# ishine/StyleTTS-ZS

Measured on AMD Instinct MI355X. Metric: synthesized audio-sec/sec (whole job) + p50 utterance latency, 3-s ref -> 5-s target, higher is better.
Workload: dtype bf16; 1 GPU; configs[2]: batch 64/GPU, 5-s targets, 2-step distilled style diffusion, CFG 5; global_batch=64, seq_len=200, parallelism=dp1 (utterance shards), spec=v0, graph=True, branch_streams=False, streams=2, schedule=pipe, stagger=0

## Files before the change

include/stzs.h:

```cpp
#ifndef STZS_H
#define STZS_H

#include <stddef.h>
#include <stdint.h>

#ifdef __cplusplus
extern "C" {
#endif

#define STZS_OK 0
#define STZS_EINVAL (-1)
#define STZS_ESHAPE (-2)
#define STZS_EDTYPE (-3)
#define STZS_EHIP (-4)

enum { STZS_F32 = 0, STZS_BF16 = 1, STZS_I32 = 2, STZS_F8 = 3  };
enum { STZS_ACT_NONE = 0, STZS_ACT_LEAKY = 1, STZS_ACT_SNAKE = 2, STZS_ACT_GELU = 3, STZS_ACT_SILU = 4 };
enum { STZS_PRO_NONE = 0, STZS_PRO_ADAIN = 1 };
#define STZS_CONV_A_DMA 8

int stzs_init(int device);
const char* stzs_strerror(int code);
int stzs_version(void);

// ... 17 lines not shown
    int32_t in_dtype, out_dtype;
    int32_t pro_mode, pro_act, epi_act, flags;
    float pro_cscale, pro_slope, epi_slope, alpha, beta, pad_f;
    void* stat_part;
    int64_t stat_ld;
    const float* x_scale;
    const float* w_scale;
    void* splitk_ws;
    unsigned int* splitk_ctr;
    int32_t splitk;
    int32_t pad_sk;
    const float* pro_part;
    int64_t pro_ld;
    int32_t pro_nch, pro_T;
    float pro_eps, pad_pp;
} stzs_conv_args;
size_t stzs_conv_splitk_workspace(int64_t rows, int32_t co_pad, int32_t splitk);
#define STZS_CONV_STAT_ROWS 64
#define STZS_CONV_W_LANE16 16
#define STZS_CONV_W_NARROW32 32
#define STZS_CONV_W_F32 64
#define STZS_CONV_LINEAR_IDS 128
#define STZS_CONV_W_FRAG32 256
#define STZS_CONV_W_X3 1024
#define STZS_CONV_ROWS 2048
#define STZS_CONV_UPS_NOISE 4096
#define STZS_CONV_MRFV_NARROW 8192
#define STZS_CONV_W_FRAG32X3 16384
#define STZS_CONV_MRFV_T128 32768
#define STZS_CONV_RING 65536
// ... 331 lines not shown
```

styletts-zs_amd/csrc/dispatch.hip:

```cpp
#include "common.hpp"

int stzs_conv1d_core(const stzs_conv_args* a, void* stream);
int stzs_mrfv_conv_launch(const stzs_conv_args& a, hipStream_t s);
int stzs_rows_gemm_launch(const stzs_conv_args& a, hipStream_t s);
int stzs_mrfx_conv_launch(const stzs_conv_args& a, hipStream_t s);

int stzs_mrfv_trio_launch(const stzs_conv_args* a, hipStream_t s);
int stzs_conv_pair_launch(const stzs_conv_args* a, hipStream_t s);

namespace {

int frag32_checks(const stzs_conv_args* a) {
    if (!a->x || !a->w || !a->y) return STZS_EINVAL;
    if (a->flags & (STZS_CONV_W_LANE16 | STZS_CONV_W_NARROW32 | STZS_CONV_W_F32 | STZS_CONV_A_DMA)) return STZS_EINVAL;
    if (a->B <= 0 || a->T_in <= 0 || a->T_out <= 0 || a->Ci <= 0 || a->Co <= 0 || a->dil <= 0) return STZS_ESHAPE;
    if (a->ci_pad < a->Ci || a->co_pad < a->Co) return STZS_ESHAPE;
    if (a->ldx % 8 || a->bsx % 8 || a->ldx < ((a->Ci + 7) / 8) * 8) return STZS_ESHAPE;
    if (!stzs_aligned(a->x, 16) || !stzs_aligned(a->w, 16) || !stzs_aligned(a->y, 16)) return STZS_EINVAL;
    if (a->pro_mode == STZS_PRO_ADAIN && (!a->pro_mean || !a->pro_rstd || !a->pro_gb)) return STZS_EINVAL;
    if (a->in_dtype == STZS_F8 || a->x_scale) return STZS_EDTYPE;
    if (a->splitk > 1) return STZS_EINVAL;
    if (a->stat_part && !stzs_aligned(a->stat_part, 8)) return STZS_EINVAL;
    return STZS_OK;
}

}

extern "C" int stzs_conv1d_group(const stzs_conv_args* a, int n, void* stream) {
    if (!a || n < 1 || n > 3) return STZS_EINVAL;
    if (n == 3 && !a[0].pro_part && !a[1].pro_part && !a[2].pro_part && (a[0].flags & STZS_CONV_W_FRAG32) &&
        (a[1].flags & STZS_CONV_W_FRAG32) && (a[2].flags & STZS_CONV_W_FRAG32) && !(a[0].flags & STZS_CONV_W_FRAG32X3) &&
        !(a[1].flags & STZS_CONV_W_FRAG32X3) && !(a[2].flags & STZS_CONV_W_FRAG32X3) && a[0].ups <= 0 && a[1].ups <= 0 &&
        a[2].ups <= 0 && frag32_checks(&a[0]) == STZS_OK && frag32_checks(&a[1]) == STZS_OK &&
        frag32_checks(&a[2]) == STZS_OK) {
        const int rc = stzs_mrfv_trio_launch(a, reinterpret_cast<hipStream_t>(stream));
        if (rc == STZS_OK) return 1;
        if (rc != STZS_ESHAPE) return rc;
    }
    if (n == 2 && !a[0].pro_part == !a[1].pro_part) {
        const int rc = stzs_conv_pair_launch(a, reinterpret_cast<hipStream_t>(stream));
        if (rc == STZS_OK) return 1;
        if (rc != STZS_ESHAPE) return rc;
    }
    for (int i = 0; i < n; ++i) {
        const int rc = stzs_conv1d(&a[i], stream);
        if (rc != STZS_OK) return rc;
    }
    return n;
}

extern "C" int stzs_conv1d(const stzs_conv_args* a, void* stream) {
    if (a && a->pro_part && (a->flags & (STZS_CONV_W_FRAG32X3 | STZS_CONV_W_FRAG32 | STZS_CONV_ROWS))) return STZS_EINVAL;
    if (a && (a->flags & STZS_CONV_W_FRAG32X3)) {
        if (!a->x || !a->w || !a->y) return STZS_EINVAL;
        if (a->flags & (STZS_CONV_W_LANE16 | STZS_CONV_W_NARROW32 | STZS_CONV_W_F32 | STZS_CONV_W_X3 | STZS_CONV_A_DMA |
                        STZS_CONV_W_FRAG32 | STZS_CONV_ROWS | STZS_CONV_UPS_NOISE))
            return STZS_EINVAL;
        if (a->B <= 0 || a->T_in <= 0 || a->T_out <= 0 || a->Ci <= 0 || a->Co <= 0 || a->dil <= 0) return STZS_ESHAPE;
        if (a->ci_pad < a->Ci || a->co_pad < a->Co || a->ldx < ((a->Ci + 7) / 8) * 8) return STZS_ESHAPE;
        if (!stzs_aligned(a->w, 16)) return STZS_EINVAL;
        if (a->pro_mode == STZS_PRO_ADAIN && (!a->pro_mean || !a->pro_rstd || !a->pro_gb)) return STZS_EINVAL;
        if (a->in_dtype == STZS_F8 || a->x_scale) return STZS_EDTYPE;
        if (a->splitk > 1) return STZS_EINVAL;
        if (a->stat_part && !stzs_aligned(a->stat_part, 8)) return STZS_EINVAL;
        return stzs_mrfx_conv_launch(*a, reinterpret_cast<hipStream_t>(stream));
    }
// ... 17 lines not shown
```

styletts-zs_amd/csrc/lnrows.hip:

```cpp
#include "conv_common.hpp"

namespace {

constexpr int LR_ROWS = 16;

STZS_DEV float sum16(float v) {
    v += dpp_f32<0x128>(v);
    v += dpp_f32<0x124>(v);
    v += dpp_f32<0x122>(v);
    v += dpp_f32<0x121>(v);
    return v;
}

template <typename TI, typename TOut, int NK, int EACT>
__global__ __launch_bounds__(NTHR) void ln_rows(const stzs_conv_args a, const stzs_rowln_args ln) {
    constexpr int K = NK * 32;
    constexpr int PITCH = K * 2 + 16;
    constexpr int NV = NK / 4;
    __shared__ __attribute__((aligned(16))) unsigned char lds[LR_ROWS * PITCH];
    const int tid = threadIdx.x, lane = tid & 63, wave = tid >> 6;
    const int nR = ln.R;
    const int r0 = blockIdx.y * LR_ROWS;
    const int ct = blockIdx.x * 4 + wave;
    const bool wact = ct * 16 < a.Co;
// ... 264 lines not shown
    const int wpg = (!split && nks <= 16) ? env_wpg : 4;
    if (a->in_dtype == STZS_BF16 && a->out_dtype == STZS_BF16) k = pick_plain<bf16_t, bf16_t>(nks, split, a->epi_act, wpg);
    else if (a->in_dtype == STZS_BF16 && a->out_dtype == STZS_F32) k = pick_plain<bf16_t, float>(nks, split, a->epi_act, wpg);
    else if (a->in_dtype == STZS_F32 && a->out_dtype == STZS_F32) k = pick_plain<float, float>(nks, split, a->epi_act, wpg);
    else return STZS_EDTYPE;
    if (!k) return STZS_EINVAL;
    dim3 grid((unsigned)((a->Co + 16 * wpg - 1) / (16 * wpg)), (unsigned)(((long)a->B * a->T_in + LR_ROWS - 1) / LR_ROWS),
              (unsigned)Z);
    hipLaunchKernelGGL(reinterpret_cast<void (*)(stzs_conv_args)>(k), grid, dim3(64 * wpg), 0, s, *a);
    STZS_LAUNCH_CHECK();
    return STZS_OK;
}

extern "C" int stzs_ln_linear(const stzs_conv_args* a, const stzs_rowln_args* ln, void* stream) {
    if (!a || !a->w || !a->y) return STZS_EINVAL;
    if (!ln) return plain_launch(a, reinterpret_cast<hipStream_t>(stream));
    if (!ln->x || ln->lens) return STZS_EINVAL;
    const bool lin = a->ks == 1 && a->stride == 1 && a->pad == 0 && a->ups == 0 && a->T_in == a->T_out &&
                     a->pro_mode == STZS_PRO_NONE && a->pro_act == STZS_ACT_NONE && !a->stat_part && !a->x_scale &&
                     !a->res && !a->gate && a->splitk <= 1;
    if (!lin || (a->flags & (STZS_CONV_W_LANE16 | STZS_CONV_W_NARROW32 | STZS_CONV_W_F32 | STZS_CONV_W_X3 |
                             STZS_CONV_W_FRAG32 | STZS_CONV_UPS_NOISE)))
        return STZS_EINVAL;
    if (a->B <= 0 || a->T_in <= 0 || a->Co <= 0 || a->Co > a->co_pad || a->co_pad % 128) return STZS_ESHAPE;
    const int C = ln->C, nk = C / 32;
    if (C != a->Ci || C != a->ci_pad || C % 32 || (nk != 4 && nk != 8 && nk != 16)) return STZS_ESHAPE;
    if ((long)ln->R != (long)a->B * a->T_in || ln->R >= (1 << 22) - LR_ROWS || ln->ldx % 8 || ln->gdiv <= 0 ||
        !stzs_aligned(ln->x, 16))
        return STZS_ESHAPE;
    if ((ln->G && (ln->gs % 8 || !stzs_aligned(ln->G, 32))) || (ln->Bt && (ln->bs % 8 || !stzs_aligned(ln->Bt, 32))))
// ... 17 lines not shown
```

styletts-zs_amd/csrc/mrfv.hip:

```cpp
#include "mrfv_kernel.hpp"

namespace {

template <int PACT, bool HR, bool HA>
void (*pick(int ks, bool one, bool al, bool wide, bool t64))(stzs_conv_args) {
    if (wide) return al ? pick_ks<PACT, HR, HA, 0, true, 2>(ks) : pick_ks<PACT, HR, HA, 0, false, 2>(ks);
    static_assert(PACT == STZS_ACT_SNAKE, "the single-chunk forms are the Snake (MRF) convs");
    if (one) return stzs_mrfv_pick_n1(ks, HR, HA, al, t64);
    if (t64)
        return al ? pick_ks<PACT, HR, HA, 0, true, 1, 64>(ks) : pick_ks<PACT, HR, HA, 0, false, 1, 64>(ks);
    return al ? pick_ks<PACT, HR, HA, 0, true>(ks) : pick_ks<PACT, HR, HA, 0, false>(ks);
}

}

int stzs_ups_conv_launch(const stzs_conv_args& a, hipStream_t s);

namespace {

int mrfv_shape(const stzs_conv_args& a) {
    const int rows_in = 128 + (a.ks - 1) * a.dil;
    if (a.stride != 1 || a.cic != 128 || a.ci_pad % 128 || a.Co % 8 || a.co_pad % BCO || rows_in > 16 * sb_rows(a.ks) ||
        a.in_dtype != STZS_BF16 || a.out_dtype != STZS_BF16 || a.gate || a.epi_act != STZS_ACT_NONE || a.ups ||
        a.refl || a.ldy % 8 || a.bsy % 8 || (a.res && (a.ldr % 8 || a.bsr % 8 || a.res_tdiv <= 0)) ||
// ... 37 lines not shown
    void (*k)(stzs_conv_args, stzs_conv_args, stzs_conv_args) =
        a[0].ci_pad == 128 ? stzs_mrfv_trio_pick_n1(R) : (R ? mrfv_trio<true, 0, 64> : mrfv_trio<false, 0, 64>);
    (void)hipFuncSetAttribute((const void*)k, hipFuncAttributeMaxDynamicSharedMemorySize, (int)lds);
    dim3 grid((unsigned)a[0].B * (unsigned)((a[0].T_out + 63) / 64), a[0].co_pad / BCO, 3);
    hipLaunchKernelGGL(k, grid, dim3(NTH), lds, s, a[0], a[1], a[2]);
    STZS_LAUNCH_CHECK();
    return STZS_OK;
}

__attribute__((visibility("hidden"))) int stzs_mrfv_conv_launch(const stzs_conv_args& a, hipStream_t s) {
    if (a.ups > 0) return stzs_ups_conv_launch(a, s);
    {
        const int rc = mrfv_shape(a);
        if (rc != STZS_OK) return rc;
    }
    void (*k)(stzs_conv_args) = nullptr;
    const bool R = a.res != nullptr, A = a.acc_in != nullptr;
    bool blk_wide = false, blk_t64 = false;
    bool wide, t64;
    snake_form(a, wide, t64);
    const long wide_tiles = (long)a.B * ((a.T_out + 127) / 128) * (a.co_pad / (2 * BCO));
    const long tiles128 = (long)a.B * ((a.T_out + 127) / 128) * (a.co_pad / BCO);
    if (a.pro_act == STZS_ACT_SNAKE) {
        const bool one = a.ci_pad == 128;
        const bool al = a.alpha != 1.f;
        k = R ? (A ? pick<STZS_ACT_SNAKE, true, true>(a.ks, one, al, wide, t64) : pick<STZS_ACT_SNAKE, true, false>(a.ks, one, al, wide, t64))
              : (A ? pick<STZS_ACT_SNAKE, false, true>(a.ks, one, al, wide, t64) : pick<STZS_ACT_SNAKE, false, false>(a.ks, one, al, wide, t64));
    } else if (!A && a.ks == 1 && a.pro_act == STZS_ACT_NONE && a.pro_mode == STZS_PRO_NONE && !a.stat_part) {
        blk_wide = a.ci_pad > 128 && a.co_pad % (2 * BCO) == 0 && wide_tiles >= 2 * stzs_cu_count() &&
                   !(a.flags & STZS_CONV_MRFV_NARROW);
        blk_t64 = !blk_wide && tiles128 < 4 * stzs_cu_count() && !(a.flags & STZS_CONV_MRFV_T128);
// ... 10 lines not shown
        blk_t64 = !blk_wide && t64_blk > 0 && tiles128 < t64_blk * stzs_cu_count() && !(a.flags & STZS_CONV_MRFV_T128);
        if (a.pro_act == STZS_ACT_LEAKY)
            k = blk_wide ? (R ? mrfv_conv<STZS_ACT_LEAKY, true, false, 3, 0, true, 2> : mrfv_conv<STZS_ACT_LEAKY, false, false, 3, 0, true, 2>)
              : blk_t64 ? (R ? mrfv_conv<STZS_ACT_LEAKY, true, false, 3, 0, true, 1, 64> : mrfv_conv<STZS_ACT_LEAKY, false, false, 3, 0, true, 1, 64>)
                         : (R ? mrfv_conv<STZS_ACT_LEAKY, true, false, 3, 0, true> : mrfv_conv<STZS_ACT_LEAKY, false, false, 3, 0, true>);
        else if (a.pro_act == STZS_ACT_NONE)
            k = blk_wide ? (R ? mrfv_conv<STZS_ACT_NONE, true, false, 3, 0, true, 2> : mrfv_conv<STZS_ACT_NONE, false, false, 3, 0, true, 2>)
              : blk_t64 ? (R ? mrfv_conv<STZS_ACT_NONE, true, false, 3, 0, true, 1, 64> : mrfv_conv<STZS_ACT_NONE, false, false, 3, 0, true, 1, 64>)
                         : (R ? mrfv_conv<STZS_ACT_NONE, true, false, 3, 0, true> : mrfv_conv<STZS_ACT_NONE, false, false, 3, 0, true>);
    }
    if (!k) return STZS_ESHAPE;
    const int BTk = (t64 || blk_t64) ? 64 : 128;
    const size_t ldsk = mrfv_lds(BTk + (a.ks - 1) * a.dil);
    (void)hipFuncSetAttribute((const void*)k, hipFuncAttributeMaxDynamicSharedMemorySize, (int)ldsk);
    dim3 grid((unsigned)a.B * (unsigned)((a.T_out + BTk - 1) / BTk), a.co_pad / (wide || blk_wide ? 2 * BCO : BCO));
    hipLaunchKernelGGL(k, grid, dim3(NTH), ldsk, s, a);
    STZS_LAUNCH_CHECK();
    return STZS_OK;
}
```

styletts-zs_amd/csrc/mrfv_kernel.hpp:

```cpp
#pragma once
#include "common.hpp"

#include <type_traits>

#ifndef STZS_MRFV_OCC
#define STZS_MRFV_OCC 2
#endif
#ifndef STZS_MRFV_OCC1
#define STZS_MRFV_OCC1 3
#endif

namespace {

constexpr int NTH = 256;
constexpr int BCO = 128;
#ifndef STZS_MRFV_P
#define STZS_MRFV_P 288
#endif
constexpr int P = STZS_MRFV_P;
constexpr int sb_rows(int ks) { return ks == 1 ? 8 : ks == 3 ? 9 : (ks == 7 ? 10 : 12); }
constexpr int sb_rows64(int ks) { return ks == 1 ? 4 : ks == 3 ? 5 : (ks == 7 ? 6 : 8); }
constexpr int SB_MAX = 12;
constexpr int CS_BYTES = 5 * 128 * 4;
constexpr bool CS_IN_PAD = P >= 288;
// ... 20 lines not shown
    for (int i = 0; i < N; ++i) asm volatile("v_add_f32_dpp %0, %0, %0 row_mirror row_mask:0xf bank_mask:0xf" : "+v"(x[i]));
}

#ifdef STZS_MRFV_PROF
__device__ unsigned long long g_mprof[8 * 16384];
#define MPROF(i, v)                                                                    \
    if (threadIdx.x == 0) {                                                            \
        const unsigned wg_ = blockIdx.y * gridDim.x + blockIdx.x;                     \
        if (wg_ < 16384) g_mprof[wg_ * 8 + (i)] = (v);                                 \
    }
#else
#define MPROF(i, v)
#endif

template <int PACT, bool HR, bool HA, int KS, int NCH, bool AL, int WPW = 1, int BT = 128>
STZS_DEV void mrfv_body(const stzs_conv_args a) {
    static_assert(WPW == 1 || (WPW == 2 && NCH != 1), "the wide form is for multi-chunk inputs");
    static_assert(BT == 128 || (BT == 64 && WPW == 1), "64-row tiles: narrow form");
    MPROF(5, __builtin_amdgcn_s_memrealtime())
    MPROF(0, __builtin_amdgcn_s_memtime())
    MPROF(7, (unsigned long long)__builtin_amdgcn_s_getreg(4 | (31 << 11)) |
                 ((unsigned long long)__builtin_amdgcn_s_getreg(0x14 | (3 << 11)) << 32))
    constexpr int NA = 2 * WPW;
    constexpr int MT = BT / 16;
    extern __shared__ __attribute__((aligned(16))) unsigned char smem[];
    constexpr int NKC = KS * 4;
    const int dil = a.dil;
    const int rows_in = BT + (KS - 1) * dil;
    auto cs = [&](int i) { return cs_at(smem, rows_in, i); };
    const int tid = threadIdx.x, lane = tid & 63, wave = tid >> 6;
    const int tpb = (a.T_out + BT - 1) / BT;
    const int nx = gridDim.x;
    const int lin = (a.flags & STZS_CONV_LINEAR_IDS) ? blockIdx.y * nx + blockIdx.x
                                                      : xcd_remap(blockIdx.y * nx + blockIdx.x, nx * gridDim.y);
    const int by = lin / nx, bx = lin - by * nx;
    const int bq = bx / tpb;
    const int t0 = (bx - bq * tpb) * BT;
    const int nchunk = NCH ? NCH : a.ci_pad >> 7;
    constexpr int SB = BT == 128 ? sb_rows(KS) : sb_rows64(KS);
    const int ct = WPW == 1 ? by : by * 2 + (wave >> 1);
    const int ow0 = WPW == 1 ? wave : (wave & 1) * 2;
    const bf16x8* Wf = reinterpret_cast<const bf16x8*>(a.w) + ((long)ct * nchunk * NKC) * 512 + ow0 * 128 + lane;
    auto wload = [&](bf16x8 (&w)[NA], int kk) {
        const bf16x8* p = Wf + (long)kk * 512;
#pragma unroll
        for (int j = 0; j < NA; ++j) w[j] = p[64 * j];
    };
    f32x4 acc[NA][MT];

// ... 283 lines not shown
                    Pp[2 * i + 1] = sq[i];
                }
            }
        }
    }
    }
#ifdef STZS_MRFV_PROF
    MPROF(3, __builtin_amdgcn_s_memtime())
    asm volatile("s_waitcnt vmcnt(0)" ::: "memory");
    MPROF(4, __builtin_amdgcn_s_memtime())
    MPROF(6, __builtin_amdgcn_s_memrealtime())
#endif
}

template <int PACT, bool HR, bool HA, int KS, int NCH, bool AL, int WPW = 1, int BT = 128>
__global__ __launch_bounds__(NTH, NCH == 1 ? STZS_MRFV_OCC1 : STZS_MRFV_OCC) void mrfv_conv(const stzs_conv_args a) {
    mrfv_body<PACT, HR, HA, KS, NCH, AL, WPW, BT>(a);
}

template <bool HR, int NCH, int BT>
__global__ __launch_bounds__(NTH, NCH == 1 ? STZS_MRFV_OCC1 : STZS_MRFV_OCC) void mrfv_trio(const stzs_conv_args a3,
                                                                                        const stzs_conv_args a7,
                                                                                        const stzs_conv_args a11) {
    if (blockIdx.z == 0)
        mrfv_body<STZS_ACT_SNAKE, HR, false, 11, NCH, false, 1, BT>(a11);
    else if (blockIdx.z == 1)
        mrfv_body<STZS_ACT_SNAKE, HR, false, 7, NCH, false, 1, BT>(a7);
    else
        mrfv_body<STZS_ACT_SNAKE, HR, false, 3, NCH, false, 1, BT>(a3);
}

template <int PACT, bool HR, bool HA, int NCH, bool AL, int WPW = 1, int BT = 128>
void (*pick_ks(int ks))(stzs_conv_args) {
    switch (ks) {
        case 3: return mrfv_conv<PACT, HR, HA, 3, NCH, AL, WPW, BT>;
        case 7: return mrfv_conv<PACT, HR, HA, 7, NCH, AL, WPW, BT>;
        case 11: return mrfv_conv<PACT, HR, HA, 11, NCH, AL, WPW, BT>;
        default: return nullptr;
    }
}

}

using mrfv_kfn = void (*)(stzs_conv_args);
mrfv_kfn stzs_mrfv_pick_n1(int ks, bool hr, bool ha, bool al, bool t64);
using mrfv_trio_kfn = void (*)(stzs_conv_args, stzs_conv_args, stzs_conv_args);
mrfv_trio_kfn stzs_mrfv_trio_pick_n1(bool hr);
```

styletts-zs_amd/csrc/norm.hip:

```cpp
#include "common.hpp"
#include "rowln.hpp"

namespace {

constexpr int STAT_ROWS = 256;
constexpr int STAT_CG = 32;

template <typename T>
__global__ __launch_bounds__(256) void chan_stats_partial(const stzs_stats_args a, int nchunk) {
    __shared__ float red[8][STAT_CG * 8][2];
    const int tid = threadIdx.x, tx = tid & 31, ty = tid >> 5;
    const int chunk = blockIdx.x, b = blockIdx.y;
    const int cv = blockIdx.z * STAT_CG + tx;
    const int c = cv * 8;
    float s[8], q[8];
#pragma unroll
    for (int j = 0; j < 8; ++j) s[j] = q[j] = 0.f;
    const int r0 = chunk * STAT_ROWS, r1 = min(a.T, r0 + STAT_ROWS);
    const T* X = reinterpret_cast<const T*>(a.x) + (long)b * a.bs;
    if (c < a.C) {
        int r = r0 + ty;
        for (; r + 24 < r1; r += 32) {
            float v[4][8];
#pragma unroll
// ... 26 lines not shown
    const int cg = blockIdx.z * STAT_CG * 8 + cl;
    if (cg < a.C) {
        float ss = 0.f, qq = 0.f;
#pragma unroll
        for (int y = 0; y < 8; ++y) {
            ss += red[y][cl][0];
            qq += red[y][cl][1];
        }
        float* P = reinterpret_cast<float*>(a.partial);
        const long o = (((long)b * nchunk + chunk) * a.C + cg) * 2;
        P[o] = ss;
        P[o + 1] = qq;
    }
}

constexpr int FIN_CH = 32;
STZS_DEV void stats_final_body(const stzs_stats_args a, int nchunk, int b, int by) {
    __shared__ double red[8][FIN_CH][2];
    const int tid = threadIdx.x, cl = tid & (FIN_CH - 1), g = tid >> 5;
    const int c = by * FIN_CH + cl;
    double s = 0.0, q = 0.0;
    if (c < a.C) {
        const float2* P = reinterpret_cast<const float2*>(a.partial) + (long)b * nchunk * a.C + c;
        int k = g;
        for (; k + 24 < nchunk; k += 32) {
            float2 v[4];
#pragma unroll
            for (int u = 0; u < 4; ++u) v[u] = P[(long)(k + 8 * u) * a.C];
#pragma unroll
            for (int u = 0; u < 4; ++u) {
                s += (double)v[u].x;
                q += (double)v[u].y;
            }
        }
        for (; k < nchunk; k += 8) {
            const float2 v = P[(long)k * a.C];
            s += (double)v.x;
            q += (double)v.y;
        }
    }
    red[g][cl][0] = s;
    red[g][cl][1] = q;
    __syncthreads();
    if (tid < FIN_CH && c < a.C) {
        s = q = 0.0;
#pragma unroll
        for (int y = 0; y < 8; ++y) {
            s += red[y][tid][0];
            q += red[y][tid][1];
        }
        float mu, rs;
        stat_finish(s, q, a.T, a.eps, mu, rs);
        a.mean[(long)b * a.stat_bs + c] = mu;
        a.rstd[(long)b * a.stat_bs + c] = rs;
    }
}

__global__ __launch_bounds__(256) void chan_stats_final(const stzs_stats_args a, int nchunk) {
    stats_final_body(a, nchunk, blockIdx.x, blockIdx.y);
}

struct StatsGroup {
    stzs_stats_args a[3];
    int nchunk[3];
};
__global__ __launch_bounds__(256) void chan_stats_final_group(const StatsGroup g) {
    const int z = blockIdx.z;
    const stzs_stats_args& a = z == 0 ? g.a[0] : (z == 1 ? g.a[1] : g.a[2]);
    if ((int)blockIdx.x >= a.B || (int)blockIdx.y * FIN_CH >= a.C) return;
    stats_final_body(a, z == 0 ? g.nchunk[0] : (z == 1 ? g.nchunk[1] : g.nchunk[2]), blockIdx.x, blockIdx.y);
}


template <typename TI, typename TO>
__global__ __launch_bounds__(256) void row_ln(const stzs_rowln_args a) {
    const long r = (long)blockIdx.x * 4 + (threadIdx.x >> 6);
    if (r >= a.R) return;
    stzs_ln::row_ln_one<TI, TO>(a, r, threadIdx.x & 63);
}

__global__ __launch_bounds__(256) void quant_rows(const stzs_quant_args a) {
    constexpr int MAXV = 4;
    const int lane = threadIdx.x & 63;
    const long r = (long)blockIdx.x * 4 + (threadIdx.x >> 6);
    if (r >= a.R) return;
// ... 126 lines not shown
```

styletts-zs_amd/stzs/_lib.py:

```python
from __future__ import annotations

import ctypes as C
import os

_HERE = os.path.dirname(os.path.abspath(__file__))
LIB_PATH = os.environ.get("STZS_LIB", os.path.join(_HERE, "libstzs_hip.so"))

F32, BF16, I32, F8 = 0, 1, 2, 3
OK, EINVAL, ESHAPE, EDTYPE, EHIP = 0, -1, -2, -3, -4
ACT_NONE, ACT_LEAKY, ACT_SNAKE, ACT_GELU, ACT_SILU = 0, 1, 2, 3, 4
PRO_NONE, PRO_ADAIN = 0, 1
CONV_STAT_ROWS = 64
CONV_W_LANE16 = 16
CONV_W_NARROW32 = 32
CONV_W_FRAG32 = 256
CONV_W_F32 = 64
CONV_W_X3 = 1024
CONV_LINEAR_IDS = 128
CONV_ROWS = 2048
CONV_UPS_NOISE = 4096
CONV_MRFV_NARROW = 8192
CONV_MRFV_T128 = 32768
CONV_RING = 65536
CONV_SK_TICKET = 131072
# ... 4 lines not shown
i32 = C.c_int32
f32 = C.c_float


class ConvArgs(C.Structure):
    _fields_ = [(n, vp) for n in ("x", "w", "bias", "y", "res", "acc_in", "gate", "pro_mean", "pro_rstd",
                                  "pro_gb", "pro_alpha")] + \
               [(n, i64) for n in ("ldx", "bsx", "ldy", "bsy", "ldr", "bsr", "lda", "bsa",
                                   "gate_bs", "stat_bs", "gb_bs", "gb_beta_off")] + \
               [(n, i32) for n in ("B", "T_in", "T_out", "Ci", "Co", "ks", "dil", "stride", "pad",
                                   "ci_pad", "co_pad", "cic", "ups", "ups_pad", "T_final", "refl", "res_tdiv",
                                   "in_dtype", "out_dtype", "pro_mode", "pro_act", "epi_act", "flags")] + \
               [(n, f32) for n in ("pro_cscale", "pro_slope", "epi_slope", "alpha", "beta", "pad_f")] + \
               [("stat_part", vp), ("stat_ld", i64), ("x_scale", vp), ("w_scale", vp),
                ("splitk_ws", vp), ("splitk_ctr", vp), ("splitk", i32), ("pad_sk", i32),
                ("pro_part", vp), ("pro_ld", i64), ("pro_nch", i32), ("pro_T", i32), ("pro_eps", f32), ("pad_pp", f32)]


class StatsArgs(C.Structure):
    _fields_ = [("x", vp), ("mean", vp), ("rstd", vp), ("partial", vp),
                ("ld", i64), ("bs", i64), ("stat_bs", i64),
                ("B", i32), ("T", i32), ("C", i32), ("dtype", i32), ("eps", f32), ("pad_f", f32)]


class RowLNArgs(C.Structure):
    _fields_ = [("x", vp), ("y", vp), ("G", vp), ("Bt", vp),
                ("ldx", i64), ("ldy", i64), ("gs", i64), ("bs", i64),
                ("R", i32), ("C", i32), ("gdiv", i32), ("in_dtype", i32), ("out_dtype", i32), ("act", i32),
                ("gadd", f32), ("eps", f32), ("slope", f32), ("pad_f", f32), ("y_scale", vp),
                ("lens", vp), ("T", i32), ("pad_t", i32)]

# ... 245 lines not shown
```

styletts-zs_amd/stzs/engine.py:

```python
from __future__ import annotations

import ctypes as C
import math
import os
from dataclasses import dataclass
from functools import partial

import numpy as np
import torch

from . import _lib as L
from .spec import Spec
from .weights import ConvW, PackedModel

_DT = {torch.float32: L.F32, torch.bfloat16: L.BF16, torch.float8_e4m3fn: L.F8}
DN_SPLITK = {}
LATENCY_DN_SPLITK = dict(ff2=4)
DN_ROWS = {}
LATENCY_DN_ROWS = dict(inp=1, qkv=1, o=1, q=1, co=1, ff1=1, ff2=4, out=1)
TE_SPLITK = 0
LATENCY_TE_SPLITK = 4
BLK_SPLITK = 0
LATENCY_BLK_SPLITK = 16

# ... 33 lines not shown
    return {k: int(n) for k, n in (kv.split("=") for kv in v.split(","))}


def _on(v):
    return v != "0"


_KNOBS = (
    ("dur_overlap", "STZS_DUR_OVERLAP", "1", lambda v: bool(int(v))),
    ("dn_splitk", "STZS_DN_SPLITK", DN_SPLITK, _table),
    ("dn_rows", "STZS_DN_ROWS", DN_ROWS, _table),
    ("te_splitk", "STZS_TE_SPLITK", TE_SPLITK, int),
    ("blk_splitk", "STZS_BLK_SPLITK", BLK_SPLITK, int),
    ("defer_stats", "STZS_DEFER_STATS", lambda eng: "1" if eng.blk_splitk else "0", _on),
    ("mrf_trio", "STZS_MRF_TRIO", "1", _on),
    ("f0n_pair", "STZS_F0N_PAIR", "1", _on),
    ("kv_fuse", "STZS_KV_FUSE", "1", _on),
    ("small_rows", "STZS_SMALL_ROWS", "1", _on),
    ("ln_fuse", "STZS_LN_FUSE", "1", _on),
    ("rows16", "STZS_ROWS16", "1", _on),
    ("rows16_split", "STZS_ROWS16_SPLIT", "1", _on),
    ("rows16_maxk", "STZS_ROWS16_MAXK", "512", int),
    ("ups_noise_fused", "STZS_UPS_NOISE", "1", _on),
    ("noise_super", "STZS_NOISE_SUPER", "1", _on),
    ("mrfx", "STZS_MRFX", "1", _on),
    ("conv_flags", "STZS_CONV_FLAGS", "0", lambda v: int(v, 0)),
)


def _rup(x, m):
# ... 72 lines not shown
    f = np.exp(-math.log(10000.0) * np.arange(half) / half)
    arg = 1000.0 * c_noise * f
    return np.concatenate([np.cos(arg), np.sin(arg)]).astype(np.float32)


class _StatsRef:

    def __init__(self, eng, part, ld, nch, T, B, mean, rstd, chunk_rows):
        self.eng, self.part, self.ld, self.nch, self.T, self.B = eng, part, ld, nch, T, B
        self.mean, self.rstd, self.chunk_rows, self.done = mean, rstd, chunk_rows, False

    def final_args(self, s):
        s.mean, s.rstd, s.partial = self.mean.data_ptr(), self.rstd.data_ptr(), self.part.data_ptr()
        s.stat_bs, s.B, s.T, s.C, s.eps = self.ld, self.B, self.T, self.ld, 1e-5
        return s

    def finalize(self):
        if not self.done:
            self.eng._raw(self.eng.lib.stzs_chan_stats_final, "chan_stats_final",
                          C.byref(self.final_args(L.StatsArgs())), self.chunk_rows)
            self.done = True

    def mean_ptr(self):
        self.finalize()
        return self.mean.data_ptr()

    def rstd_ptr(self):
        self.finalize()
        return self.rstd.data_ptr()

# ... 125 lines not shown
            e1 = torch.cuda.Event(enable_timing=True)
            e0.record()
        L.check(fn(*args, self.stream()), what)
        if rec:
            e1.record()
            flop, byt = cost() if callable(cost) else (float(cost[0]), float(cost[1]))
            tm["rec"].append((what, e0, e1, flop, byt, shape, self.stage))

    def _raw(self, fn, what, *args):
        self._call(fn, None, what, args=args)

    def conv(self, cw: ConvW, x: Act, y: Act, *, T_out=None, pad=0, dil=1, stride=1, pro=None, pro_act=L.ACT_NONE,
             pro_slope=0.0, pro_alpha=None, cscale=1.0, res: Act = None, res_tdiv=1, acc_in: Act = None,
             alpha=1.0, beta=0.0, gate=None, gate_bs=0, epi_act=L.ACT_NONE, epi_slope=0.0, ups_pad=0,
             T_final=0, refl=0, flags=0, stats_key=None, x_scale=None, post_ln=None, pre_ln=None, splitk=0, rows=0,
             attn=None, collect=None, what="conv"):
        a, pro_ref = self._conv_fill(cw, x, y, what, T_out=T_out, pad=pad, dil=dil, stride=stride, pro=pro,
                                     pro_act=pro_act, pro_slope=pro_slope, pro_alpha=pro_alpha, cscale=cscale, res=res,
                                     res_tdiv=res_tdiv, acc_in=acc_in, alpha=alpha, beta=beta, gate=gate,
                                     gate_bs=gate_bs, epi_act=epi_act, epi_slope=epi_slope, ups_pad=ups_pad,
                                     T_final=T_final, refl=refl, x_scale=x_scale)
        rows = self._conv_route(a, cw, x, y, flags, rows, cscale, res, stats_key)
        if rows > 1 or splitk > 1:
            self._conv_splitk(a, cw, x, splitk, rows, collect, what)
        if pro_ref is not None:
            self._conv_stats_in(a, cw, pro_ref, pre_ln)
        st = self._conv_stats_out(a, cw, y, stats_key, collect) if stats_key is not None else None
        fn, args, fused = self._conv_entry(a, cw, x, res, res_tdiv, gate, pre_ln, st)
        if collect is not None:
            assert len(args) == 1 and pre_ln is None and post_ln is None and attn is None, what
            collect.append(a)
        else:
            if pre_ln is not None and not fused:
                self._call(self.lib.stzs_row_layernorm, pre_ln, what + ".ln", cost=_ln_cost(pre_ln))
            rec = {} if self.timer is None else dict(
                shape=(cw.ks, dil, a.T_out, cw.Co),
                cost=partial(_conv_cost, cw, x, y, a.T_out, res, acc_in, pre_ln if fused else None))
            self._call(fn, a, what, args=args, **rec)
        if post_ln is not None:
            self._call(self.lib.stzs_row_layernorm, post_ln, what + ".ln", cost=_ln_cost(post_ln))
        if attn is not None:
            self.attention(*attn)
# ... 114 lines not shown
            a.splitk_ctr = self._counters("sk_ctr", nb // (splitk * 32768)).data_ptr()
        elif splitk > 1 and _conv_generic(a.flags, cw):
            tiles = x.B * ((a.T_out + 127) // 128) * (cw.co_pad // 128)
            a.splitk = splitk
            gs = f".g{len(collect)}" if collect is not None else ""
            a.splitk_ws = self._scratch("csk_ws" + gs, tiles * splitk * 16384).data_ptr()
            a.splitk_ctr = self._counters("csk_ctr" + gs, tiles).data_ptr()

    def _conv_stats_in(self, a, cw, pro_ref, pre_ln):
        if _conv_generic(a.flags, cw) and pre_ln is None and pro_ref.nch <= 8:
            a.pro_part, a.pro_ld, a.pro_nch, a.pro_T, a.pro_eps = pro_ref.part.data_ptr(), pro_ref.ld, pro_ref.nch, \
                pro_ref.T, 1e-5
        else:
            a.pro_mean, a.pro_rstd = pro_ref.mean_ptr(), pro_ref.rstd_ptr()

    def _conv_stats_out(self, a, cw, y, stats_key, collect):
        Cc = _rup(cw.Co, 8)
        ntile = (a.T_out + L.CONV_STAT_ROWS - 1) // L.CONV_STAT_ROWS
        defer = collect is not None or (self.defer_stats and ntile <= 8)
        slab = self._scratch("stat_slab." + stats_key, y.B * ntile * Cc * 2, 1024) if defer else \
            self._scratch("stat_slab", y.B * ntile * Cc * 2)
        a.stat_part, a.stat_ld = slab.data_ptr(), Cc
        return (slab, Cc, self.buf(stats_key + ".m", (y.B, Cc), torch.float32),
                self.buf(stats_key + ".r", (y.B, Cc), torch.float32), defer, ntile)

    def _conv_entry(self, a, cw, x, res, res_tdiv, gate, pre_ln, st):
        if not (a.flags & L.CONV_ROWS):
            return self.lib.stzs_conv1d, (C.byref(a),), False
        nk = cw.ci_pad // 32
        if pre_ln is not None:
            fused = a.splitk <= 1 and res is None and gate is None and \
                st is None and pre_ln.C == cw.Ci == cw.ci_pad and nk in (4, 8, 16) and pre_ln.out_dtype == L.BF16 and \
                pre_ln.act == L.ACT_NONE and (pre_ln.x or 0) % 16 == 0 and pre_ln.ldx % 8 == 0 and \
                pre_ln.gdiv > 0 and pre_ln.R < (1 << 22) - 16 and \
# ... 987 lines not shown
        arr = (L.ConvArgs * len(args))(*args)
        rc = self.lib.stzs_conv1d_group(arr, len(args), self.stream())
        if rc < 0:
            L.check(rc, what)
        self.launches += rc

    def _finalize_group(self, refs):
        arr = (L.StatsArgs * len(refs))()
        for s, r in zip(arr, refs):
            r.final_args(s)
        assert len({r.chunk_rows for r in refs}) == 1
        self._raw(self.lib.stzs_chan_stats_final_group, "chan_stats_final_group", arr, len(refs), refs[0].chunk_rows)
        for r in refs:
            r.done = True

    def _rb_c1(self, lw, x: Act, y: Act, st, gbd, ng, stats_key, collect=None):
        k, dil = lw["k"], lw["dil"]
        o1, c1 = ng.offsets[lw["n1"]]
        return self.conv(lw["c1"], x, y, pad=dil * (k - 1) // 2, dil=dil,
                         pro=(*st, gbd.data_ptr() + o1 * 4, ng.total, c1), pro_act=L.ACT_SNAKE, pro_alpha=lw["a1"],
                         stats_key=stats_key, collect=collect, what="rb.c1")[1]

    def _rb_c2(self, lw, x: Act, y: Act, st, res: Act, gbd, ng, **kw):
        o2, c2 = ng.offsets[lw["n2"]]
        return self.conv(lw["c2"], x, y, pad=(lw["k"] - 1) // 2, pro=(*st, gbd.data_ptr() + o2 * 4, ng.total, c2),
                         pro_act=L.ACT_SNAKE, pro_alpha=lw["a2"], res=res, what="rb.c2", **kw)

    def _mrf_trio(self, x: Act, i, gbd, ng):
        S, W = self.spec, self.W
        B, T, c = x.B, x.T, x.C
        dt = x.t.dtype
        nk = len(S.rb_kernels)
        xs = self.act(f"gen.xs{i}", B, T, c, dt)
        t1 = [self.act(f"gen.t1_{i}.{j}", B, T, c, dt) for j in range(nk)]
        bufs = [(self.act(f"gen.ba{i}.{j}", B, T, c, dt), self.act(f"gen.bb{i}.{j}", B, T, c, dt)) for j in range(nk)]
        mx, rx, sb = self.stats(x, f"gen.sx{i}")
# ... 13 lines not shown
            grp = []
            outs = [bufs[j][0] if cur[j] is not bufs[j][0] else bufs[j][1] for j in range(nk)]
            st2 = [self._rb_c2(res[m], t1[j], outs[j], (*st1[j][:2], sb), cur[j], gbd, ng,
                               stats_key=f"gen.sc{i}.{j}.{m % 2}", collect=grp)[1] for j, res in enumerate(W.rb[i])]
            self._launch_group(grp, "rb.c2")
            self._finalize_group([st[0].ref for st in st2])
            for j in range(nk):
                cur[j], (cm[j], cr[j], _) = outs[j], st2[j]
        return xs

    def _mrf_trio_on(self, x: Act, i) -> bool:
        rb = self.W.rb[i]
        return (self.mrf_trio and self.timer is None and x.B <= 4 and tuple(self.spec.rb_kernels) == (3, 7, 11) and
                len({len(res) for res in rb}) == 1 and all(r["k"] == k for res, k in zip(rb, (3, 7, 11)) for r in res))

    def mrf(self, x: Act, i, gbd, ng):
        S, W = self.spec, self.W
        if self._mrf_trio_on(x, i):
            return self._mrf_trio(x, i, gbd, ng)
        B, T, c = x.B, x.T, x.C
        dt = x.t.dtype
        xs = self.act(f"gen.xs{i}", B, T, c, dt)
        bufA = self.act(f"gen.ba{i}", B, T, c, dt)
        bufB = self.act(f"gen.bb{i}", B, T, c, dt)
        t1 = self.act(f"gen.t1_{i}", B, T, c, dt)
        mx, rx, sb = self.stats(x, f"gen.sx{i}")
        nk = len(S.rb_kernels)
        for j, res in enumerate(W.rb[i]):
            cur, cm, cr = x, mx, rx
            for m, lw in enumerate(res):
                tm, tr, _ = self._rb_c1(lw, cur, t1, (cm, cr, sb), gbd, ng, f"gen.st{i}")
                last = m == len(res) - 1
                out = xs if last else (bufA if cur is not bufA else bufB)
                r2 = self._rb_c2(lw, t1, out, (tm, tr, sb), cur, gbd, ng, alpha=(1.0 / nk) if last else 1.0,
# ... 112 lines not shown
```

Baseline: 19500 audio-s/s.

## Piggyback channel-stats finalization onto next MRF conv launch as rider blocks

Adds 'rider' fields to the conv args so that an MRF-branch frag32 conv launch carries extra blocks that finalize the pending channel statistics of the previous conv in another branch, instead of launching a separate stats-final kernel. A new interleaved MRF schedule for batches above 4 issues the three kernel branches round-robin so each conv finalizes the prior one's stats, and stats are deferred into per-key slabs. This removes standalone small finalize launches and the serial gaps around them, at the cost of extra grid blocks, a wider kernel signature and some added checks.

After: 19370 audio-s/s. Within noise of the previous version (-0.7%).

```diff
diff --git a/include/stzs.h b/include/stzs.h
--- a/include/stzs.h
+++ b/include/stzs.h
@@ -55,6 +55,12 @@
     int64_t pro_ld;
     int32_t pro_nch, pro_T;
     float pro_eps, pad_pp;
+    const void* rider_partial;
+    float* rider_mean;
+    float* rider_rstd;
+    int64_t rider_stat_bs;
+    int32_t rider_B, rider_T, rider_C, rider_chunk_rows;
+    float rider_eps, pad_rd;
 } stzs_conv_args;
 size_t stzs_conv_splitk_workspace(int64_t rows, int32_t co_pad, int32_t splitk);
 #define STZS_CONV_STAT_ROWS 64
diff --git a/styletts-zs_amd/csrc/dispatch.hip b/styletts-zs_amd/csrc/dispatch.hip
--- a/styletts-zs_amd/csrc/dispatch.hip
+++ b/styletts-zs_amd/csrc/dispatch.hip
@@ -24,10 +24,23 @@
     return STZS_OK;
 }
 
+bool rider_set(const stzs_conv_args* a) { return a->rider_partial || a->rider_mean || a->rider_rstd; }
+
+int rider_checks(const stzs_conv_args* a) {
+    if (!a->rider_partial || !a->rider_mean || !a->rider_rstd) return STZS_EINVAL;
+    if (!stzs_aligned(a->rider_partial, 8) || !stzs_aligned(a->rider_mean, 8) || !stzs_aligned(a->rider_rstd, 8))
+        return STZS_EINVAL;
+    if (a->rider_chunk_rows <= 0 || a->rider_stat_bs < a->rider_C) return STZS_EINVAL;
+    if (a->rider_B <= 0 || a->rider_T <= 0 || a->rider_C <= 0) return STZS_ESHAPE;
+    return STZS_OK;
+}
+
 }
 
 extern "C" int stzs_conv1d_group(const stzs_conv_args* a, int n, void* stream) {
     if (!a || n < 1 || n > 3) return STZS_EINVAL;
+    for (int i = 0; i < n; ++i)
+        if (rider_set(&a[i])) return STZS_EINVAL;
     if (n == 3 && !a[0].pro_part && !a[1].pro_part && !a[2].pro_part && (a[0].flags & STZS_CONV_W_FRAG32) &&
         (a[1].flags & STZS_CONV_W_FRAG32) && (a[2].flags & STZS_CONV_W_FRAG32) && !(a[0].flags & STZS_CONV_W_FRAG32X3) &&
         !(a[1].flags & STZS_CONV_W_FRAG32X3) && !(a[2].flags & STZS_CONV_W_FRAG32X3) && a[0].ups <= 0 && a[1].ups <= 0 &&
@@ -50,6 +63,12 @@
 }
 
 extern "C" int stzs_conv1d(const stzs_conv_args* a, void* stream) {
+    if (a && rider_set(a) && a->B > 0 && a->T_in > 0 && a->T_out > 0 && a->Ci > 0 && a->Co > 0) {
+        if (!(a->flags & STZS_CONV_W_FRAG32) || (a->flags & (STZS_CONV_W_FRAG32X3 | STZS_CONV_ROWS)) || a->ups > 0)
+            return STZS_EINVAL;
+        const int rc = rider_checks(a);
+        if (rc != STZS_OK) return rc;
+    }
     if (a && a->pro_part && (a->flags & (STZS_CONV_W_FRAG32X3 | STZS_CONV_W_FRAG32 | STZS_CONV_ROWS))) return STZS_EINVAL;
     if (a && (a->flags & STZS_CONV_W_FRAG32X3)) {
         if (!a->x || !a->w || !a->y) return STZS_EINVAL;
diff --git a/styletts-zs_amd/csrc/lnrows.hip b/styletts-zs_amd/csrc/lnrows.hip
--- a/styletts-zs_amd/csrc/lnrows.hip
+++ b/styletts-zs_amd/csrc/lnrows.hip
@@ -302,6 +302,7 @@
 
 extern "C" int stzs_ln_linear(const stzs_conv_args* a, const stzs_rowln_args* ln, void* stream) {
     if (!a || !a->w || !a->y) return STZS_EINVAL;
+    if (a->rider_partial || a->rider_mean || a->rider_rstd) return STZS_EINVAL;
     if (!ln) return plain_launch(a, reinterpret_cast<hipStream_t>(stream));
     if (!ln->x || ln->lens) return STZS_EINVAL;
     const bool lin = a->ks == 1 && a->stride == 1 && a->pad == 0 && a->ups == 0 && a->T_in == a->T_out &&
diff --git a/styletts-zs_amd/csrc/mrfv.hip b/styletts-zs_amd/csrc/mrfv.hip
--- a/styletts-zs_amd/csrc/mrfv.hip
+++ b/styletts-zs_amd/csrc/mrfv.hip
@@ -3,7 +3,7 @@
 namespace {
 
 template <int PACT, bool HR, bool HA>
-void (*pick(int ks, bool one, bool al, bool wide, bool t64))(stzs_conv_args) {
+mrfv_kfn pick(int ks, bool one, bool al, bool wide, bool t64) {
     if (wide) return al ? pick_ks<PACT, HR, HA, 0, true, 2>(ks) : pick_ks<PACT, HR, HA, 0, false, 2>(ks);
     static_assert(PACT == STZS_ACT_SNAKE, "the single-chunk forms are the Snake (MRF) convs");
     if (one) return stzs_mrfv_pick_n1(ks, HR, HA, al, t64);
@@ -75,7 +75,7 @@
         const int rc = mrfv_shape(a);
         if (rc != STZS_OK) return rc;
     }
-    void (*k)(stzs_conv_args) = nullptr;
+    mrfv_kfn k = nullptr;
     const bool R = a.res != nullptr, A = a.acc_in != nullptr;
     bool blk_wide = false, blk_t64 = false;
     bool wide, t64;
@@ -116,7 +116,17 @@
     const size_t ldsk = mrfv_lds(BTk + (a.ks - 1) * a.dil);
     (void)hipFuncSetAttribute((const void*)k, hipFuncAttributeMaxDynamicSharedMemorySize, (int)ldsk);
     dim3 grid((unsigned)a.B * (unsigned)((a.T_out + BTk - 1) / BTk), a.co_pad / (wide || blk_wide ? 2 * BCO : BCO));
-    hipLaunchKernelGGL(k, grid, dim3(NTH), ldsk, s, a);
+    int rx = 0;
+    if (a.rider_partial) {
+        static_assert(FIN_LDS <= CS_ROWS * P, "the smallest tile holds the rider's LDS scratch");
+        if (ldsk < (size_t)FIN_LDS) return STZS_ESHAPE;
+        const long nrb = (long)a.rider_B * ((a.rider_C + FIN_CH - 1) / FIN_CH);
+        const long per_row = (nrb + grid.y - 1) / grid.y;
+        if ((long)grid.x + per_row > 0x7fffffffL) return STZS_ESHAPE;
+        rx = (int)per_row;
+        grid.x += rx;
+    }
+    hipLaunchKernelGGL(k, grid, dim3(NTH), ldsk, s, a, rx);
     STZS_LAUNCH_CHECK();
     return STZS_OK;
 }
diff --git a/styletts-zs_amd/csrc/mrfv_kernel.hpp b/styletts-zs_amd/csrc/mrfv_kernel.hpp
--- a/styletts-zs_amd/csrc/mrfv_kernel.hpp
+++ b/styletts-zs_amd/csrc/mrfv_kernel.hpp
@@ -1,5 +1,6 @@
 #pragma once
 #include "common.hpp"
+#include "stats_final.hpp"
 
 #include <type_traits>
 
@@ -58,9 +59,32 @@
 #endif
 
 template <int PACT, bool HR, bool HA, int KS, int NCH, bool AL, int WPW = 1, int BT = 128>
-STZS_DEV void mrfv_body(const stzs_conv_args a) {
+STZS_DEV void mrfv_body(const stzs_conv_args a, const int rx) {
     static_assert(WPW == 1 || (WPW == 2 && NCH != 1), "the wide form is for multi-chunk inputs");
     static_assert(BT == 128 || (BT == 64 && WPW == 1), "64-row tiles: narrow form");
+    if ((int)blockIdx.x < rx) {
+        extern __shared__ __attribute__((aligned(16))) unsigned char smem[];
+        const int ncb = (a.rider_C + FIN_CH - 1) / FIN_CH;
+        const int rb = blockIdx.y * rx + blockIdx.x;
+        const int b = rb / ncb;
+        if (b >= a.rider_B) return;
+        stzs_stats_args s;
+        s.x = nullptr;
+        s.mean = a.rider_mean;
+        s.rstd = a.rider_rstd;
+        s.partial = const_cast<void*>(a.rider_partial);
+        s.ld = s.bs = 0;
+        s.stat_bs = a.rider_stat_bs;
+        s.B = a.rider_B;
+        s.T = a.rider_T;
+        s.C = a.rider_C;
+        s.dtype = 0;
+        s.eps = a.rider_eps;
+        s.pad_f = 0.f;
+        stats_final_body(s, (a.rider_T + a.rider_chunk_rows - 1) / a.rider_chunk_rows, b, rb - b * ncb,
+                         reinterpret_cast<double(*)[FIN_CH][2]>(smem));
+        return;
+    }
     MPROF(5, __builtin_amdgcn_s_memrealtime())
     MPROF(0, __builtin_amdgcn_s_memtime())
     MPROF(7, (unsigned long long)__builtin_amdgcn_s_getreg(4 | (31 << 11)) |
@@ -74,9 +98,9 @@
     auto cs = [&](int i) { return cs_at(smem, rows_in, i); };
     const int tid = threadIdx.x, lane = tid & 63, wave = tid >> 6;
     const int tpb = (a.T_out + BT - 1) / BT;
-    const int nx = gridDim.x;
-    const int lin = (a.flags & STZS_CONV_LINEAR_IDS) ? blockIdx.y * nx + blockIdx.x
-                                                      : xcd_remap(blockIdx.y * nx + blockIdx.x, nx * gridDim.y);
+    const int nx = (int)gridDim.x - rx;
+    const int lin0 = blockIdx.y * nx + ((int)blockIdx.x - rx);
+    const int lin = (a.flags & STZS_CONV_LINEAR_IDS) ? lin0 : xcd_remap(lin0, nx * gridDim.y);
     const int by = lin / nx, bx = lin - by * nx;
     const int bq = bx / tpb;
     const int t0 = (bx - bq * tpb) * BT;
@@ -390,8 +414,9 @@
 }
 
 template <int PACT, bool HR, bool HA, int KS, int NCH, bool AL, int WPW = 1, int BT = 128>
-__global__ __launch_bounds__(NTH, NCH == 1 ? STZS_MRFV_OCC1 : STZS_MRFV_OCC) void mrfv_conv(const stzs_conv_args a) {
-    mrfv_body<PACT, HR, HA, KS, NCH, AL, WPW, BT>(a);
+__global__ __launch_bounds__(NTH, NCH == 1 ? STZS_MRFV_OCC1 : STZS_MRFV_OCC) void mrfv_conv(const stzs_conv_args a,
+                                                                                        const int rx) {
+    mrfv_body<PACT, HR, HA, KS, NCH, AL, WPW, BT>(a, rx);
 }
 
 template <bool HR, int NCH, int BT>
@@ -399,15 +424,15 @@
                                                                                         const stzs_conv_args a7,
                                                                                         const stzs_conv_args a11) {
     if (blockIdx.z == 0)
-        mrfv_body<STZS_ACT_SNAKE, HR, false, 11, NCH, false, 1, BT>(a11);
+        mrfv_body<STZS_ACT_SNAKE, HR, false, 11, NCH, false, 1, BT>(a11, 0);
     else if (blockIdx.z == 1)
-        mrfv_body<STZS_ACT_SNAKE, HR, false, 7, NCH, false, 1, BT>(a7);
+        mrfv_body<STZS_ACT_SNAKE, HR, false, 7, NCH, false, 1, BT>(a7, 0);
     else
-        mrfv_body<STZS_ACT_SNAKE, HR, false, 3, NCH, false, 1, BT>(a3);
+        mrfv_body<STZS_ACT_SNAKE, HR, false, 3, NCH, false, 1, BT>(a3, 0);
 }
 
 template <int PACT, bool HR, bool HA, int NCH, bool AL, int WPW = 1, int BT = 128>
-void (*pick_ks(int ks))(stzs_conv_args) {
+void (*pick_ks(int ks))(stzs_conv_args, int) {
     switch (ks) {
         case 3: return mrfv_conv<PACT, HR, HA, 3, NCH, AL, WPW, BT>;
         case 7: return mrfv_conv<PACT, HR, HA, 7, NCH, AL, WPW, BT>;
@@ -418,7 +443,7 @@
 
 }
 
-using mrfv_kfn = void (*)(stzs_conv_args);
+using mrfv_kfn = void (*)(stzs_conv_args, int);
 mrfv_kfn stzs_mrfv_pick_n1(int ks, bool hr, bool ha, bool al, bool t64);
 using mrfv_trio_kfn = void (*)(stzs_conv_args, stzs_conv_args, stzs_conv_args);
 mrfv_trio_kfn stzs_mrfv_trio_pick_n1(bool hr);
diff --git a/styletts-zs_amd/csrc/norm.hip b/styletts-zs_amd/csrc/norm.hip
--- a/styletts-zs_amd/csrc/norm.hip
+++ b/styletts-zs_amd/csrc/norm.hip
@@ -1,5 +1,6 @@
 #include "common.hpp"
 #include "rowln.hpp"
+#include "stats_final.hpp"
 
 namespace {
 
@@ -64,50 +65,9 @@
     }
 }
 
-constexpr int FIN_CH = 32;
-STZS_DEV void stats_final_body(const stzs_stats_args a, int nchunk, int b, int by) {
+__global__ __launch_bounds__(256) void chan_stats_final(const stzs_stats_args a, int nchunk) {
     __shared__ double red[8][FIN_CH][2];
-    const int tid = threadIdx.x, cl = tid & (FIN_CH - 1), g = tid >> 5;
-    const int c = by * FIN_CH + cl;
-    double s = 0.0, q = 0.0;
-    if (c < a.C) {
-        const float2* P = reinterpret_cast<const float2*>(a.partial) + (long)b * nchunk * a.C + c;
-        int k = g;
-        for (; k + 24 < nchunk; k += 32) {
-            float2 v[4];
-#pragma unroll
-            for (int u = 0; u < 4; ++u) v[u] = P[(long)(k + 8 * u) * a.C];
-#pragma unroll
-            for (int u = 0; u < 4; ++u) {
-                s += (double)v[u].x;
-                q += (double)v[u].y;
-            }
-        }
-        for (; k < nchunk; k += 8) {
-            const float2 v = P[(long)k * a.C];
-            s += (double)v.x;
-            q += (double)v.y;
-        }
-    }
-    red[g][cl][0] = s;
-    red[g][cl][1] = q;
-    __syncthreads();
-    if (tid < FIN_CH && c < a.C) {
-        s = q = 0.0;
-#pragma unroll
-        for (int y = 0; y < 8; ++y) {
-            s += red[y][tid][0];
-            q += red[y][tid][1];
-        }
-        float mu, rs;
-        stat_finish(s, q, a.T, a.eps, mu, rs);
-        a.mean[(long)b * a.stat_bs + c] = mu;
-        a.rstd[(long)b * a.stat_bs + c] = rs;
-    }
-}
-
-__global__ __launch_bounds__(256) void chan_stats_final(const stzs_stats_args a, int nchunk) {
-    stats_final_body(a, nchunk, blockIdx.x, blockIdx.y);
+    stats_final_body(a, nchunk, blockIdx.x, blockIdx.y, red);
 }
 
 struct StatsGroup {
@@ -115,10 +75,11 @@
     int nchunk[3];
 };
 __global__ __launch_bounds__(256) void chan_stats_final_group(const StatsGroup g) {
+    __shared__ double red[8][FIN_CH][2];
     const int z = blockIdx.z;
     const stzs_stats_args& a = z == 0 ? g.a[0] : (z == 1 ? g.a[1] : g.a[2]);
     if ((int)blockIdx.x >= a.B || (int)blockIdx.y * FIN_CH >= a.C) return;
-    stats_final_body(a, z == 0 ? g.nchunk[0] : (z == 1 ? g.nchunk[1] : g.nchunk[2]), blockIdx.x, blockIdx.y);
+    stats_final_body(a, z == 0 ? g.nchunk[0] : (z == 1 ? g.nchunk[1] : g.nchunk[2]), blockIdx.x, blockIdx.y, red);
 }
 
 
diff --git a/styletts-zs_amd/csrc/stats_final.hpp b/styletts-zs_amd/csrc/stats_final.hpp
--- /dev/null
+++ b/styletts-zs_amd/csrc/stats_final.hpp
@@ -0,0 +1,49 @@
+#pragma once
+#include "common.hpp"
+
+namespace {
+
+constexpr int FIN_CH = 32;
+constexpr int FIN_LDS = 8 * FIN_CH * 2 * (int)sizeof(double);
+
+STZS_DEV void stats_final_body(const stzs_stats_args a, int nchunk, int b, int by, double (*red)[FIN_CH][2]) {
+    const int tid = threadIdx.x, cl = tid & (FIN_CH - 1), g = tid >> 5;
+    const int c = by * FIN_CH + cl;
+    double s = 0.0, q = 0.0;
+    if (c < a.C) {
+        const float2* P = reinterpret_cast<const float2*>(a.partial) + (long)b * nchunk * a.C + c;
+        int k = g;
+        for (; k + 24 < nchunk; k += 32) {
+            float2 v[4];
+#pragma unroll
+            for (int u = 0; u < 4; ++u) v[u] = P[(long)(k + 8 * u) * a.C];
+#pragma unroll
+            for (int u = 0; u < 4; ++u) {
+                s += (double)v[u].x;
+                q += (double)v[u].y;
+            }
+        }
+        for (; k < nchunk; k += 8) {
+            const float2 v = P[(long)k * a.C];
+            s += (double)v.x;
+            q += (double)v.y;
+        }
+    }
+    red[g][cl][0] = s;
+    red[g][cl][1] = q;
+    __syncthreads();
+    if (tid < FIN_CH && c < a.C) {
+        s = q = 0.0;
+#pragma unroll
+        for (int y = 0; y < 8; ++y) {
+            s += red[y][tid][0];
+            q += red[y][tid][1];
+        }
+        float mu, rs;
+        stat_finish(s, q, a.T, a.eps, mu, rs);
+        a.mean[(long)b * a.stat_bs + c] = mu;
+        a.rstd[(long)b * a.stat_bs + c] = rs;
+    }
+}
+
+}
diff --git a/styletts-zs_amd/stzs/_lib.py b/styletts-zs_amd/stzs/_lib.py
--- a/styletts-zs_amd/stzs/_lib.py
+++ b/styletts-zs_amd/stzs/_lib.py
@@ -42,7 +42,10 @@
                [(n, f32) for n in ("pro_cscale", "pro_slope", "epi_slope", "alpha", "beta", "pad_f")] + \
                [("stat_part", vp), ("stat_ld", i64), ("x_scale", vp), ("w_scale", vp),
                 ("splitk_ws", vp), ("splitk_ctr", vp), ("splitk", i32), ("pad_sk", i32),
-                ("pro_part", vp), ("pro_ld", i64), ("pro_nch", i32), ("pro_T", i32), ("pro_eps", f32), ("pad_pp", f32)]
+                ("pro_part", vp), ("pro_ld", i64), ("pro_nch", i32), ("pro_T", i32), ("pro_eps", f32), ("pad_pp", f32),
+                ("rider_partial", vp), ("rider_mean", vp), ("rider_rstd", vp), ("rider_stat_bs", i64),
+                ("rider_B", i32), ("rider_T", i32), ("rider_C", i32), ("rider_chunk_rows", i32),
+                ("rider_eps", f32), ("pad_rd", f32)]
 
 
 class StatsArgs(C.Structure):
diff --git a/styletts-zs_amd/stzs/engine.py b/styletts-zs_amd/stzs/engine.py
--- a/styletts-zs_amd/stzs/engine.py
+++ b/styletts-zs_amd/stzs/engine.py
@@ -71,6 +71,7 @@
     ("blk_splitk", "STZS_BLK_SPLITK", BLK_SPLITK, int),
     ("defer_stats", "STZS_DEFER_STATS", lambda eng: "1" if eng.blk_splitk else "0", _on),
     ("mrf_trio", "STZS_MRF_TRIO", "1", _on),
+    ("mrf_rider", "STZS_MRF_RIDER", "1", _on),
     ("f0n_pair", "STZS_F0N_PAIR", "1", _on),
     ("kv_fuse", "STZS_KV_FUSE", "1", _on),
     ("small_rows", "STZS_SMALL_ROWS", "1", _on),
@@ -173,6 +174,13 @@
         s.mean, s.rstd, s.partial = self.mean.data_ptr(), self.rstd.data_ptr(), self.part.data_ptr()
         s.stat_bs, s.B, s.T, s.C, s.eps = self.ld, self.B, self.T, self.ld, 1e-5
         return s
+
+    def ride(self, a):
+        assert not self.done
+        a.rider_partial, a.rider_mean, a.rider_rstd = self.part.data_ptr(), self.mean.data_ptr(), self.rstd.data_ptr()
+        a.rider_stat_bs, a.rider_B, a.rider_T, a.rider_C = self.ld, self.B, self.T, self.ld
+        a.rider_chunk_rows, a.rider_eps = self.chunk_rows, 1e-5
+        self.done = True
 
     def finalize(self):
         if not self.done:
@@ -328,7 +336,7 @@
              pro_slope=0.0, pro_alpha=None, cscale=1.0, res: Act = None, res_tdiv=1, acc_in: Act = None,
              alpha=1.0, beta=0.0, gate=None, gate_bs=0, epi_act=L.ACT_NONE, epi_slope=0.0, ups_pad=0,
              T_final=0, refl=0, flags=0, stats_key=None, x_scale=None, post_ln=None, pre_ln=None, splitk=0, rows=0,
-             attn=None, collect=None, what="conv"):
+             attn=None, collect=None, rider=None, defer_stats=False, what="conv"):
         a, pro_ref = self._conv_fill(cw, x, y, what, T_out=T_out, pad=pad, dil=dil, stride=stride, pro=pro,
                                      pro_act=pro_act, pro_slope=pro_slope, pro_alpha=pro_alpha, cscale=cscale, res=res,
                                      res_tdiv=res_tdiv, acc_in=acc_in, alpha=alpha, beta=beta, gate=gate,
@@ -339,7 +347,10 @@
             self._conv_splitk(a, cw, x, splitk, rows, collect, what)
         if pro_ref is not None:
             self._conv_stats_in(a, cw, pro_ref, pre_ln)
-        st = self._conv_stats_out(a, cw, y, stats_key, collect) if stats_key is not None else None
+        st = self._conv_stats_out(a, cw, y, stats_key, collect, defer_stats) if stats_key is not None else None
+        if rider is not None:
+            assert collect is None, what
+            rider.ride(a)
         fn, args, fused = self._conv_entry(a, cw, x, res, res_tdiv, gate, pre_ln, st)
         if collect is not None:
             assert len(args) == 1 and pre_ln is None and post_ln is None and attn is None, what
@@ -484,10 +495,10 @@
         else:
             a.pro_mean, a.pro_rstd = pro_ref.mean_ptr(), pro_ref.rstd_ptr()
 
-    def _conv_stats_out(self, a, cw, y, stats_key, collect):
+    def _conv_stats_out(self, a, cw, y, stats_key, collect, defer=False):
         Cc = _rup(cw.Co, 8)
         ntile = (a.T_out + L.CONV_STAT_ROWS - 1) // L.CONV_STAT_ROWS
-        defer = collect is not None or (self.defer_stats and ntile <= 8)
+        defer = defer or collect is not None or (self.defer_stats and ntile <= 8)
         slab = self._scratch("stat_slab." + stats_key, y.B * ntile * Cc * 2, 1024) if defer else \
             self._scratch("stat_slab", y.B * ntile * Cc * 2)
         a.stat_part, a.stat_ld = slab.data_ptr(), Cc
@@ -1505,12 +1516,12 @@
         for r in refs:
             r.done = True
 
-    def _rb_c1(self, lw, x: Act, y: Act, st, gbd, ng, stats_key, collect=None):
+    def _rb_c1(self, lw, x: Act, y: Act, st, gbd, ng, stats_key, **kw):
         k, dil = lw["k"], lw["dil"]
         o1, c1 = ng.offsets[lw["n1"]]
         return self.conv(lw["c1"], x, y, pad=dil * (k - 1) // 2, dil=dil,
                          pro=(*st, gbd.data_ptr() + o1 * 4, ng.total, c1), pro_act=L.ACT_SNAKE, pro_alpha=lw["a1"],
-                         stats_key=stats_key, collect=collect, what="rb.c1")[1]
+                         stats_key=stats_key, what="rb.c1", **kw)[1]
 
     def _rb_c2(self, lw, x: Act, y: Act, st, res: Act, gbd, ng, **kw):
         o2, c2 = ng.offsets[lw["n2"]]
@@ -1554,10 +1565,54 @@
         return (self.mrf_trio and self.timer is None and x.B <= 4 and tuple(self.spec.rb_kernels) == (3, 7, 11) and
                 len({len(res) for res in rb}) == 1 and all(r["k"] == k for res, k in zip(rb, (3, 7, 11)) for r in res))
 
+    def _mrf_riders(self, x: Act, i, gbd, ng):
+        S, W = self.spec, self.W
+        B, T, c = x.B, x.T, x.C
+        dt = x.t.dtype
+        nk = len(S.rb_kernels)
+        xs = self.act(f"gen.xs{i}", B, T, c, dt)
+        t1 = [self.act(f"gen.t1_{i}.{j}", B, T, c, dt) for j in range(nk)]
+        bufs = [(self.act(f"gen.ba{i}.{j}", B, T, c, dt), self.act(f"gen.bb{i}.{j}", B, T, c, dt)) for j in range(nk)]
+        mx, rx, sb = self.stats(x, f"gen.sx{i}")
+        cur, cm, cr = [x] * nk, [mx] * nk, [rx] * nk
+        pend = []
+
+        def ride():
+            return dict(rider=pend.pop() if pend else None, defer_stats=True)
+
+        nl = len(W.rb[i][0])
+        for m in range(nl):
+            st1 = []
+            for j, res in enumerate(W.rb[i]):
+                st1.append(self._rb_c1(res[m], cur[j], t1[j], (cm[j], cr[j], sb), gbd, ng, f"gen.st{i}.{j}", **ride()))
+                pend.append(st1[j][0].ref)
+            if m == nl - 1:
+                for j, res in enumerate(W.rb[i]):
+                    self._rb_c2(res[m], t1[j], xs, (*st1[j][:2], sb), cur[j], gbd, ng, alpha=1.0 / nk,
+                                acc_in=(xs if j > 0 else None), beta=1.0, **ride())
+                break
+            outs = [bufs[j][0] if cur[j] is not bufs[j][0] else bufs[j][1] for j in range(nk)]
+            for j, res in enumerate(W.rb[i]):
+                _, (cm[j], cr[j], _) = self._rb_c2(res[m], t1[j], outs[j], (*st1[j][:2], sb), cur[j], gbd, ng,
+                                                   stats_key=f"gen.sc{i}.{j}.{m % 2}", **ride())
+                pend.append(cm[j].ref)
+                cur[j] = outs[j]
+        assert not pend
+        return xs
+
+    def _mrf_riders_on(self, x: Act, i) -> bool:
+        rb = self.W.rb[i]
+        return (self.mrf_rider and x.B > 4 and x.t.dtype == torch.bfloat16 and len(rb) >= 2 and
+                len({len(res) for res in rb}) == 1 and
+                all(getattr(cw, "frag32", False) and cw.wx3 is None and cw.w32 is None
+                    for res in rb for lw in res for cw in (lw["c1"], lw["c2"])))
+
     def mrf(self, x: Act, i, gbd, ng):
         S, W = self.spec, self.W
         if self._mrf_trio_on(x, i):
             return self._mrf_trio(x, i, gbd, ng)
+        if self._mrf_riders_on(x, i):
+            return self._mrf_riders(x, i, gbd, ng)
         B, T, c = x.B, x.T, x.C
         dt = x.t.dtype
         xs = self.act(f"gen.xs{i}", B, T, c, dt)
```
